# GaodeRender/triangle-splatting

Hardware: AMD Instinct MI355X
Metric: fwd+bwd Mpixels/sec @ 1M triangles, 1920x1080; achieved HBM GB/s (higher is better)
Workload: dtype f32

## Files before the change

triangle-splatting_amd/csrc/api.hip:

```cpp
#pragma GCC visibility push(default)
#include "../../include/ts2d.h"
#ifdef TS2D_LAB
#include "ts2d_lab.h"
#endif
#pragma GCC visibility pop
#include "ts2d_api.h"
#include <atomic>
#include <chrono>
#include <cstdarg>
#include <cstdio>
#include <cstring>
#include <mutex>
#include <string>
#include <vector>

namespace
{
thread_local std::string g_err;

struct ProfRow { std::string name; double ms = 0; int64_t launches = 0; };
struct ProfPending { int row; hipEvent_t a, b; };
std::mutex g_prof_mu;
bool g_prof_on = false;
std::string g_prof_only;
// ... 62 lines not shown
    a.rich_info = flags & TS2D_FLAG_RICH_INFO; a.use_shs = flags & TS2D_FLAG_USE_SHS;
    a.back_culling = flags & TS2D_FLAG_BACK_CULLING;
    a.tan_fovx = cam->tan_fovx; a.tan_fovy = cam->tan_fovy;
    a.viewmatrix = cam->viewmatrix; a.projmatrix = cam->projmatrix; a.campos = cam->campos;
    a.vertex = geom->vertex; a.shs = geom->shs; a.feature = geom->feature; a.opacity = geom->opacity;
    return a;
}

RenderArgs make_render(const ts2d_camera *cam, const ts2d_geometry *geom, uint32_t flags)
{
    RenderArgs r;
    r.W = cam->width; r.H = cam->height; r.C = geom->C;
    r.grid_x = (cam->width + TS_TILE - 1) / TS_TILE; r.grid_y = (cam->height + TS_TILE - 1) / TS_TILE;
    r.gamma = geom->gamma; r.background_depth = geom->background_depth;
    r.background_depth_dev = geom->background_depth_dev;
    r.background = geom->background;
    r.rich_info = flags & TS2D_FLAG_RICH_INFO;
    r.block_masks = block_masks_in_keys(cam, flags);
#ifdef TS2D_LAB
    if (g_lab_kernel_cull) r.block_masks = false;
#endif
    return r;
}

inline void cpu_relax()
{
#if defined(__x86_64__) || defined(__i386__)
    __builtin_ia32_pause();
#elif defined(__aarch64__)
    asm volatile("yield" ::: "memory");
#endif
}

struct CapacityHint { int dev, variant, W, H; unsigned long long key; double per_triangle; unsigned long long stamp; };
thread_local unsigned long long t_hint_key = 0;
std::atomic<unsigned long long> g_speculative_overflows{0};
std::mutex g_hint_mu;
std::vector<CapacityHint> g_hints;
unsigned long long g_hint_clock = 0;

void record_instance_count(int variant, int W, int H, int P, unsigned long long n)
{
    int dev = 0;
    if (P <= 0 || hipGetDevice(&dev) != hipSuccess) return;
    const double per = (double)n / (double)P;
    std::lock_guard<std::mutex> lk(g_hint_mu);
    CapacityHint *slot = nullptr;
    for (auto &h : g_hints)
        if (h.dev == dev && h.variant == variant && h.W == W && h.H == H && h.key == t_hint_key) slot = &h;
    if (!slot)
    {
        if (g_hints.size() < 32) { g_hints.push_back({dev, variant, W, H, t_hint_key, 0.0, 0}); slot = &g_hints.back(); }
        else
        {
            slot = &g_hints[0];
            for (auto &h : g_hints)
                if (h.stamp < slot->stamp) slot = &h;
            *slot = {dev, variant, W, H, t_hint_key, 0.0, 0};
        }
    }
    slot->per_triangle = per > 0.97 * slot->per_triangle ? per : 0.97 * slot->per_triangle;
    slot->stamp = ++g_hint_clock;
}

int read_instance_count(const ts2d_camera *cam, const ts2d_geometry *geom, uint32_t flags, const ts2d_state *state, const EarlyCount *early,
                        hipStream_t s, int64_t *num_rendered)
{
    if (int rc = wait_instance_count(geom->P, state, early, s, num_rendered)) return rc;
    record_instance_count((flags & TS2D_FLAG_3D) ? 3 : 2, cam->width, cam->height, geom->P, (unsigned long long)*num_rendered);
    return TS2D_OK;
}

int forward_bin_impl(const ts2d_camera *cam, const ts2d_geometry *geom, uint32_t flags, int32_t *radii, const ts2d_state *state, hipStream_t s,
                     const EarlyCount *early)
{
    const int P = geom->P;
    GeometryStateView g;
    ts_carve_geometry((char *)state->geometry, P, g);
    const PreprocessArgs a = make_pre(cam, geom, flags);
    {
        ProfScope ps("preprocess_fwd", s);
        if (flags & TS2D_FLAG_3D) ts_launch_preprocess3d_fwd(a, radii, g, s);
        else ts_launch_preprocess_fwd(a, radii, g, s);
    }
    TS_CHECK(flags, s, "preprocess_fwd");
    return ts_order_triangles(flags, g, P, early, s);
}

int forward_render_impl(const ts2d_camera *cam, const ts2d_geometry *geom, uint32_t flags, int64_t N, bool count_on_device,
                        const ts2d_state *state, const ts2d_forward_out *out, hipStream_t s)
{
    const bool rich = flags & TS2D_FLAG_RICH_INFO;
    const int P = geom->P, W = cam->width, H = cam->height;
    GeometryStateView g{};
    BinningStateView b{};
    ImageStateView im{};
    if (P > 0) ts_carve_geometry((char *)state->geometry, P, g);
    if (N > 0)
    {
        ts_carve_binning((char *)state->binning, ts_binning_capacity(state->binning_bytes, W, H), W, H, b);
        if (!count_on_device) ts_binning_set_count(b, N);
    }
    ts_carve_image((char *)state->image, W, H, im);
    const RenderArgs r = make_render(cam, geom, flags);
    const int ntiles = r.grid_x * r.grid_y;
    const unsigned long long *n_dev = count_on_device ? ts_instance_count_dev(g, P) : nullptr;

    QuadMaskArgs quad{(flags & TS2D_FLAG_3D) ? 3 : 2, fmaxf(0.0f, 2.0f * geom->gamma), cam->tan_fovx, cam->tan_fovy, W, H, 1.0f / (float)W, 1.0f / (float)H,
                      block_masks_in_keys(cam, flags) ? 1 : 0};
#ifdef TS2D_LAB
    if (g_lab_all_quadrants) quad.variant = 0;
#endif
    if (int rc = ts_order_instances(flags, P, r.grid_x, ntiles, g, b, im, rich ? out->contrib_sum : nullptr, rich ? out->contrib_max : nullptr, N, n_dev,
                                    quad, s))
        return rc;
    {
        ProfScope ps("render_fwd", s);
        if (flags & TS2D_FLAG_3D)
            ts_launch_render3d_fwd_group(r, cam->tan_fovx, cam->tan_fovy, g, b, im, out->out_feature, out->depth, out->normal,
// ... 53 lines not shown
    if (row < 0) return;
    (void)hipEventRecord(b, s);
    std::lock_guard<std::mutex> lk(g_prof_mu);
    g_prof_pending.push_back({row, a, b});
}

bool acquire_early_count(EarlyCount &e)
{
    constexpr int SLOTS = 64, MAXDEV = 16;
    static unsigned long long *ring = [] {
        void *p = nullptr;
        return hipHostMalloc(&p, (size_t)MAXDEV * SLOTS * sizeof(unsigned long long), hipHostMallocPortable | hipHostMallocMapped | hipHostMallocCoherent) == hipSuccess
                   ? (unsigned long long *)p : nullptr;
    }();
    static hipEvent_t events[MAXDEV][SLOTS] = {};
    static std::atomic<unsigned> next{0};
    static std::mutex mu;
    int dev = 0;
    if (!ring || hipGetDevice(&dev) != hipSuccess || dev < 0 || dev >= MAXDEV) return false;
    const unsigned i = next.fetch_add(1) % SLOTS;
    {
        std::lock_guard<std::mutex> lk(mu);
#ifndef TS2D_COUNT_EVENT_FLAGS
#define TS2D_COUNT_EVENT_FLAGS (hipEventDisableTiming | hipEventBlockingSync)
#endif
        if (!events[dev][i] && hipEventCreateWithFlags(&events[dev][i], TS2D_COUNT_EVENT_FLAGS) != hipSuccess) return false;
    }
    e.host = ring + (size_t)dev * SLOTS + i;
    e.ev = events[dev][i];
    __atomic_store_n(e.host, ~0ull, __ATOMIC_RELEASE);
    return true;
}

int wait_instance_count(int P, const ts2d_state *state, const EarlyCount *early, hipStream_t s, int64_t *num_rendered)
{
    unsigned long long n = ~0ull;
    if (early)
    {
        const auto t0 = std::chrono::steady_clock::now();
        for (unsigned spin = 0;; spin++)
        {
            n = __atomic_load_n(early->host, __ATOMIC_ACQUIRE);
            if (n != ~0ull) break;
            cpu_relax();
            if ((spin & 63u) == 63u && std::chrono::steady_clock::now() - t0 > std::chrono::microseconds(250)) break;
        }
        if (n == ~0ull)
        {
            const hipError_t q = hipEventSynchronize(early->ev);
            if (q != hipSuccess) return ts_fail(TS2D_ERR_HIP, "waiting for the instance count: %s", hipGetErrorString(q));
            n = __atomic_load_n(early->host, __ATOMIC_ACQUIRE);
            if (n == ~0ull) return ts_fail(TS2D_ERR_HIP, "the instance count was not published");
        }
    }
    else
    {
        GeometryStateView g;
        ts_carve_geometry((char *)state->geometry, P, g);
        TS_HIP(hipMemcpyAsync(&n, ts_instance_count_dev(g, P), sizeof(n), hipMemcpyDeviceToHost, s));
        TS_HIP(hipStreamSynchronize(s));
    }
    if (n > 0x7fffffffull)
        return ts_fail(TS2D_ERR_CAPACITY, "%llu tile instances exceed the 2^31 - 1 the instance list can address", n);
    *num_rendered = (int64_t)n;
    return TS2D_OK;
}

int ts_order_triangles(uint32_t flags, const GeometryStateView &g, int P, const EarlyCount *early, hipStream_t s)
{
    {
        ProfScope ps("depth_census", s);
        ts_sort_by_depth_begin(g, P, early ? early->host : nullptr, s);
    }
    if (early) TS_HIP(hipEventRecord(early->ev, s));
    { ProfScope ps("depth_sort", s); ts_sort_by_depth_finish(g, P, s); }
    TS_CHECK(flags, s, "depth_sort");
    { ProfScope ps("scan", s); ts_scan_offsets(g, P, s); }
    TS_CHECK(flags, s, "scan");
    return TS2D_OK;
}

int ts_order_instances(uint32_t flags, int P, int grid_x, int ntiles, const GeometryStateView &g, const BinningStateView &b, const ImageStateView &im,
                       float *contrib_sum, float *contrib_max, int64_t N, const unsigned long long *n_dev, const QuadMaskArgs &quad, hipStream_t s)
{
    if (P > 0)
    {
        { ProfScope ps("emit_keys", s); ts_launch_emit_keys(P, grid_x, ntiles, g, b, im, contrib_sum, contrib_max, n_dev ? N : -1, im.status, quad, s); }
        TS_CHECK(flags, s, "emit_keys");
    }
    else ts_launch_zero_words((uint32_t *)im.ranges, 2 * (size_t)ntiles, s);
    if (N > 0)
    {
        { ProfScope ps("tile_sort", s); ts_sort_pairs(b, N, n_dev, ntiles, s); }
        TS_CHECK(flags, s, "tile_sort");
        { ProfScope ps("tile_ranges", s); ts_launch_tile_ranges(N, n_dev, ntiles, b, im, s); }
        TS_CHECK(flags, s, "tile_ranges");
    }
    return TS2D_OK;
}

extern "C" {

const char *ts2d_version(void) { return "ts2d 0.1 (gfx950)"; }
const char *ts2d_last_error(void) { return g_err.c_str(); }

size_t ts2d_geometry_state_bytes(int32_t P)
{
    GeometryStateView v;
// ... 57 lines not shown
int ts2d_forward_render(const ts2d_camera *cam, const ts2d_geometry *geom, uint32_t flags, int64_t N,
                        const ts2d_state *state, const ts2d_forward_out *out, void *stream)
{
    if (int rc = check_forward_args(cam, geom, flags, N, state, out)) return rc;
    return forward_render_impl(cam, geom, flags, N, false, state, out, (hipStream_t)stream);
}

int ts2d_forward(const ts2d_camera *cam, const ts2d_geometry *geom, uint32_t flags, int32_t *radii, const ts2d_state *state,
                 int64_t instance_capacity, const ts2d_forward_out *out, void *stream)
{
    if (int rc = check_forward_args(cam, geom, flags, instance_capacity, state, out)) return rc;
    hipStream_t s = (hipStream_t)stream;
    if (geom->P == 0) return forward_render_impl(cam, geom, flags, 0, false, state, out, s);
    if (!radii) return ts_fail(TS2D_ERR_INVALID, "radii is null");
    if (instance_capacity <= 0) return ts_fail(TS2D_ERR_INVALID, "instance_capacity must be positive");
    if (int rc = forward_bin_impl(cam, geom, flags, radii, state, s, nullptr)) return rc;
    return forward_render_impl(cam, geom, flags, instance_capacity, true, state, out, s);
}

int ts2d_forward_speculative(const ts2d_camera *cam, const ts2d_geometry *geom, uint32_t flags, int32_t *radii, const ts2d_state *state,
                             const ts2d_forward_out *out, int64_t *num_rendered, void *stream)
{
    if (!num_rendered) return ts_fail(TS2D_ERR_INVALID, "null num_rendered");
    *num_rendered = 0;
    if (int rc = check_forward_args(cam, geom, flags, 0, state, out)) return rc;
    hipStream_t s = (hipStream_t)stream;
    const int P = geom->P, W = cam->width, H = cam->height;
    if (P == 0) return forward_render_impl(cam, geom, flags, 0, false, state, out, s);
    if (!radii) return ts_fail(TS2D_ERR_INVALID, "radii is null");
    int64_t cap = state->binning ? ts_binning_capacity(state->binning_bytes, W, H) : 0;
    if (state->binning && cap <= 0) return ts_fail(TS2D_ERR_CAPACITY, "binning state buffer too small for any instance (pass NULL to size it from num_rendered)");
    EarlyCount early;
    const bool have_early = acquire_early_count(early);
    if (int rc = forward_bin_impl(cam, geom, flags, radii, state, s, have_early ? &early : nullptr)) return rc;
    if (cap > 0)
    {
        if (int rc = forward_render_impl(cam, geom, flags, cap, true, state, out, s)) return rc;
    }
    if (int rc = read_instance_count(cam, geom, flags, state, have_early ? &early : nullptr, s, num_rendered)) return rc;
    if (cap > 0 && *num_rendered > cap) g_speculative_overflows.fetch_add(1, std::memory_order_relaxed);
    return TS2D_OK;
}

void ts2d_set_capacity_hint_key(uint64_t key) { t_hint_key = key; }
uint64_t ts2d_speculative_overflow_count(void) { return g_speculative_overflows.load(std::memory_order_relaxed); }

int ts2d_forward_status(const ts2d_state *state, int32_t P, int32_t width, int32_t height, int32_t *overflowed, int64_t *num_rendered,
                        void *stream)
{
    if (!state || !state->image || !overflowed || !num_rendered) return ts_fail(TS2D_ERR_INVALID, "null pointer");
    hipStream_t s = (hipStream_t)stream;
    *overflowed = 0;
    *num_rendered = 0;
    if (P <= 0) return TS2D_OK;
    if (!state->geometry) return ts_fail(TS2D_ERR_INVALID, "null geometry state");
    GeometryStateView g{};
    ImageStateView im{};
    ts_carve_geometry((char *)state->geometry, P, g);
    ts_carve_image((char *)state->image, width, height, im);
    unsigned long long n = 0;
    TS_HIP(hipMemcpyAsync(overflowed, im.status, sizeof(int32_t), hipMemcpyDeviceToHost, s));
    TS_HIP(hipMemcpyAsync(&n, ts_instance_count_dev(g, P), sizeof(n), hipMemcpyDeviceToHost, s));
    TS_HIP(hipStreamSynchronize(s));
    *num_rendered = (int64_t)n;
    return TS2D_OK;
}

int ts2d_backward(const ts2d_camera *cam, const ts2d_geometry *geom, uint32_t flags, int64_t N, const int32_t *radii,
                  const ts2d_state *state, const ts2d_loss_grads *loss, void *scratch, size_t scratch_bytes,
                  const ts2d_backward_out *out, void *stream)
{
    return ts2d_backward_ranged(cam, geom, flags, N, radii, state, loss, scratch, scratch_bytes, out, 1, nullptr, stream);
// ... 186 lines not shown
    case 13: src = im.n_contrib; bytes = (size_t)W * H * 4; break;
    case 14: src = im.final_T; bytes = (size_t)W * H * 4; break;
    case 15: src = b.k[(b.passes & 1) ^ 1]; bytes = (size_t)N * 4; break;
    case 16: src = b.v[(b.passes & 1) ^ 1]; bytes = (size_t)N * 4; break;
    case 17:
    {
        uint32_t top_const = 0;
        if (P > 0)
        {
            TS_HIP(hipMemcpyAsync(&top_const, g.top_const, 4, hipMemcpyDeviceToHost, s));
            TS_HIP(hipStreamSynchronize(s));
        }
        src = top_const ? g.sv[0] : g.sv[1];
        bytes = (size_t)P * 4;
        break;
    }
    case 18: src = g.rec; bytes = (size_t)P * TS_REC_FLOATS * 4; break;
    default: return ts_fail(TS2D_ERR_INVALID, "unknown field %d", field);
    }
    if (dst_bytes < bytes) return ts_fail(TS2D_ERR_CAPACITY, "dst too small");
    if (bytes)
    {
        TS_HIP(hipMemcpyAsync(dst, src, bytes, hipMemcpyDeviceToHost, s));
        TS_HIP(hipStreamSynchronize(s));
    }
    return TS2D_OK;
}

void ts2d_lab_force_ticket_passes(int on) { ts_force_ticket_passes(on != 0); }
void ts2d_lab_force_all_quadrants(int on) { g_lab_all_quadrants = on != 0; }
void ts2d_lab_force_kernel_cull(int on) { g_lab_kernel_cull = on != 0; }
void ts2d_lab_force_depth_pass4(int on) { ts_force_depth_pass4(on != 0); }
void ts2d_lab_depth_split(int mode, int bucket_cap) { ts_lab_depth_split(mode, bucket_cap); }
#endif

void ts2d_profile_enable(int on)
{
    std::lock_guard<std::mutex> lk(g_prof_mu);
    g_prof_on = on != 0;
}
void ts2d_profile_only(const char *name)
{
    std::lock_guard<std::mutex> lk(g_prof_mu);
    g_prof_only = name ? name : "";
}
void ts2d_profile_reset(void)
{
    std::lock_guard<std::mutex> lk(g_prof_mu);
    prof_drain();
    g_prof_rows.clear();
}
int ts2d_profile_read(int32_t index, char *name, size_t name_bytes, double *total_ms, int64_t *launches)
{
    std::lock_guard<std::mutex> lk(g_prof_mu);
    prof_drain();
    if (index < 0 || (size_t)index >= g_prof_rows.size()) return TS2D_ERR_INVALID;
    const ProfRow &r = g_prof_rows[index];
    if (name && name_bytes) { strncpy(name, r.name.c_str(), name_bytes - 1); name[name_bytes - 1] = 0; }
    if (total_ms) *total_ms = r.ms;
    if (launches) *launches = r.launches;
    return TS2D_OK;
}
}
```

triangle-splatting_amd/csrc/depth_order.hip:

```cpp
#include "ts2d_radix.h"

namespace
{
bool g_force_pass4 = false;

template <int CH>
__global__ void __launch_bounds__(256) rs_hist_census_direct_kernel(const uint32_t *__restrict__ keys, int64_t n, uint32_t mask, RadixScratchView r,
                                                                     uint32_t *__restrict__ acc, DepthCensus census)
{
    __shared__ uint32_t bins[NB];
    __shared__ unsigned long long csum[4];
    __shared__ uint32_t cor[4], cand[4];
    const int t = threadIdx.x, chunk = rs_chunk_of_block(r.chunks);
    if (chunk < 0) return;
    bins[t] = 0u;
    __syncthreads();
    const int64_t base = (int64_t)chunk * CH;
    KeyCensus mine;
#pragma unroll
    for (int b = 0; b < CH / 256; b++)
    {
        const int64_t i = base + 256 * b + t;
        if (i < n)
        {
// ... 538 lines not shown
    {
        const DepthSplit ds = depth_split_of(g);
        const dim3 grid((unsigned)g.rs.chunks);
        if (P < DSPL_SMALL_BELOW) hipLaunchKernelGGL(depth_split_sample_kernel<DSPL_SAMPLES_SMALL>, dim3(NB - 1), dim3(256), 0, s, P, g, ds);
        else hipLaunchKernelGGL(depth_split_sample_kernel<DSPL_SAMPLES>, dim3(NB - 1), dim3(256), 0, s, P, g, ds);
        TS_WITH_CHUNK(g.rs.chunk,
                      hipLaunchKernelGGL((depth_split_hist_kernel<CH>), grid, dim3(256), 0, s, (int64_t)P, g, g.rs, g.rs.slabacc[0], ds);
                      hipLaunchKernelGGL((depth_split_scatter_kernel<CH>), grid, dim3(256), 0, s, (int64_t)P, g, g.rs, (const uint32_t *)g.rs.slabacc[0], ds, host_out))
        return;
    }
    DepthCensus c;
    c.tiles_touched = g.tiles_touched;
    c.chunk_sum = (unsigned long long *)g.blocksum;
    c.chunk_or = g.tiles_sorted;
    c.chunk_and = g.offsets;
    c.n_out = (unsigned long long *)g.blocksum + (P + SB - 1) / SB;
    c.host_out = host_out;
    c.top_const = g.top_const;
    c.force_varying = g_force_pass4 ? 0xFF000000u : 0u;
    const dim3 grid((unsigned)g.rs.chunks);
    const uint32_t *keys = (const uint32_t *)g.depth;
    const unsigned long long *no_count = nullptr;
    const uint32_t *no_vals = nullptr, *no_skip = nullptr;
    if (form == DepthForm::LsdTickets)
    {
        TS_WITH_CHUNK(g.rs.chunk, hipLaunchKernelGGL((rs_hist_kernel<true, CH>), grid, dim3(256), 0, s, keys, (int64_t)P, no_count, 0, 0xFFu, g.rs, c, no_skip))
        return;
    }
    TS_WITH_CHUNK(g.rs.chunk,
                  hipLaunchKernelGGL((rs_hist_census_direct_kernel<CH>), grid, dim3(256), 0, s, keys, (int64_t)P, 0xFFu, g.rs, g.rs.slabacc[0], c);
                  hipLaunchKernelGGL((rs_scatter_kernel<true, CH, true, true>), grid, dim3(256), 0, s, keys, no_vals, g.sk[0], g.sv[0], (int64_t)P, no_count, 0, 8,
                                     g.rs, no_skip, (const uint32_t *)g.rs.slabacc[0], g.rs.slabacc[1], c))
}
void ts_sort_by_depth_finish(const GeometryStateView &g, int32_t P, hipStream_t s)
{
    if (P <= 0) return;
    switch (depth_form(P, g.rs))
    {
    case DepthForm::OneLaunch: return;
    case DepthForm::Split:
        if (P < DB_SMALL_BELOW)
            hipLaunchKernelGGL(depth_bucket_sort_kernel<DB_SMALL_WAVES>, dim3(NB), dim3(64 * DB_SMALL_WAVES), 0, s, P, g, depth_split_of(g),
                               min(g_depth_bucket_cap, 64 * DB_SMALL_WAVES * DB_KB));
        else hipLaunchKernelGGL(depth_bucket_sort_kernel<DB_WAVES>, dim3(NB), dim3(64 * DB_WAVES), 0, s, P, g, depth_split_of(g), g_depth_bucket_cap);
        return;
    case DepthForm::LsdTickets:
        ts_radix_scatter((const uint32_t *)g.depth, nullptr, g.sk[0], g.sv[0], P, nullptr, 0, 8, g.rs, s);
        ts_radix_pass(g.sk[0], g.sv[0], g.sk[1], g.sv[1], P, nullptr, 8, 8, g.rs, s);
        ts_radix_pass(g.sk[1], g.sv[1], g.sk[0], g.sv[0], P, nullptr, 16, 8, g.rs, s);
        ts_radix_pass(g.sk[0], g.sv[0], g.sk[1], g.sv[1], P, nullptr, 24, 8, g.rs, s, g.top_const);
        return;
    case DepthForm::LsdDirect:
        ts_radix_pass_direct(g.sk[0], g.sv[0], g.sk[1], g.sv[1], P, nullptr, 8, 8, g.rs, 1, s);
        ts_radix_pass_direct(g.sk[1], g.sv[1], g.sk[0], g.sv[0], P, nullptr, 16, 8, g.rs, 0, s);
        ts_radix_pass_direct(g.sk[0], g.sv[0], g.sk[1], g.sv[1], P, nullptr, 24, 8, g.rs, 1, s, g.top_const);
        return;
    }
}

bool ts_scan_two_level(int32_t P) { return ts_radix_tickets_forced() || (P + SB - 1) / SB > 2048; }
void ts_scan_offsets(const GeometryStateView &g, int32_t P, hipStream_t s)
{
    if (P <= 0) return;
    switch (depth_form(P, g.rs))
    {
    case DepthForm::OneLaunch:
    case DepthForm::Split: return;
    case DepthForm::LsdDirect:
    case DepthForm::LsdTickets: break;
    }
    hipLaunchKernelGGL(gather_blocksum_kernel, dim3((unsigned)((P + SB - 1) / SB)), dim3(256), 0, s, P, g, ts_scan_two_level(P));
}

void ts_force_depth_pass4(bool on) { g_force_pass4 = on; }
void ts_lab_depth_split(int mode, int bucket_cap)
{
    g_depth_split_mode = mode;
    g_depth_bucket_cap = bucket_cap > 0 && bucket_cap < DB_CAP ? bucket_cap : DB_CAP;
}
```

triangle-splatting_amd/csrc/ts2d_api.h:

```cpp
#ifndef TS2D_API_H
#define TS2D_API_H

#include "../../include/ts2d.h"
#include "ts2d_common.h"

#pragma GCC visibility push(hidden)
int ts_fail(int code, const char *fmt, ...) __attribute__((format(printf, 2, 3)));

#define TS_HIP(expr)                                                                                                   \
    do                                                                                                                 \
    {                                                                                                                  \
        hipError_t e_ = (expr);                                                                                        \
        if (e_ != hipSuccess) return ts_fail(TS2D_ERR_HIP, "%s failed: %s", #expr, hipGetErrorString(e_));           \
    } while (0)

#define TS_CHECK(flags, stream, what)                                                                                  \
    do                                                                                                                 \
    {                                                                                                                  \
        hipError_t e_ = hipGetLastError();                                                                             \
        if (e_ == hipSuccess && ((flags)&TS2D_FLAG_DEBUG)) e_ = hipStreamSynchronize(stream);                          \
        if (e_ != hipSuccess) return ts_fail(TS2D_ERR_HIP, "%s: %s", what, hipGetErrorString(e_));                     \
    } while (0)

struct ProfScope
{
    hipStream_t s;
    int row = -1;
    hipEvent_t a = nullptr, b = nullptr;
    ProfScope(const char *name, hipStream_t stream);
    ~ProfScope();
};

struct EarlyCount
{
    unsigned long long *host = nullptr;
    hipEvent_t ev = nullptr;
};
bool acquire_early_count(EarlyCount &e);
int wait_instance_count(int P, const ts2d_state *state, const EarlyCount *early, hipStream_t s, int64_t *num_rendered);

int ts_order_triangles(uint32_t flags, const GeometryStateView &g, int P, const EarlyCount *early, hipStream_t s);
int ts_order_instances(uint32_t flags, int P, int grid_x, int ntiles, const GeometryStateView &g, const BinningStateView &b, const ImageStateView &im,
                       float *contrib_sum, float *contrib_max, int64_t N, const unsigned long long *n_dev, const QuadMaskArgs &quad, hipStream_t s);

#pragma GCC visibility pop
#endif
```

triangle-splatting_amd/csrc/ts2d_common.h:

```cpp
#pragma once
#include <hip/hip_runtime.h>
#include <stddef.h>
#include <stdint.h>

#define TS_TILE 16
#define TS_ALIGN 256

#define TS_REC_FLOATS 16

#define TS_ID_BITS 28
#define TS_ID_MASK 0x0FFFFFFFu
#define TS_GRAD_FLOATS 16

#ifndef TS_RS_CHUNK
#define TS_RS_CHUNK 4096
#endif
#define TS_RS_CHUNK_MID 2048
#define TS_RS_CHUNK_SMALL 1024
#define TS_RS_SMALL_BELOW 2500000
static inline int ts_instance_chunk(size_t n) { return n <= (size_t)TS_RS_SMALL_BELOW ? TS_RS_CHUNK_SMALL : TS_RS_CHUNK; }
static inline int ts_depth_chunk(size_t n) { return n <= (size_t)TS_RS_SMALL_BELOW ? TS_RS_CHUNK_SMALL : TS_RS_CHUNK_MID; }
#define TS_RS_BINS 256
#define TS_RS_TICKET_EXTRA 8
struct RadixScratchView
// ... 138 lines not shown
    }
    return lo;
}

static inline void ts_binning_set_count(BinningStateView &v, int64_t n)
{
    v.rs.chunks = (int)((n + v.rs.chunk - 1) / v.rs.chunk);
    v.rs.slabs = (v.rs.chunks + 63) / 64;
}

static inline size_t ts_carve_image(char *base, int32_t W, int32_t H, ImageStateView &v)
{
    char *p = base;
    int gx = (W + TS_TILE - 1) / TS_TILE, gy = (H + TS_TILE - 1) / TS_TILE;
    ts_carve(p, v.ranges, (size_t)gx * gy);
    ts_carve(p, v.n_contrib, (size_t)W * H);
    ts_carve(p, v.final_T, (size_t)W * H);
    ts_carve(p, v.status, (size_t)4);
    return (size_t)(p - base) + TS_ALIGN;
}

struct PreprocessArgs
{
    int W, H, P, D, M, C;
    int grid_x, grid_y;
    bool rich_info, use_shs, back_culling;
    float tan_fovx, tan_fovy;
    const float *viewmatrix, *projmatrix, *campos;
    const float *vertex, *shs, *feature, *opacity;
};

void ts_launch_preprocess_fwd(const PreprocessArgs &a, int32_t *radii, const GeometryStateView &g, hipStream_t s);
void ts_sort_by_depth_begin(const GeometryStateView &g, int32_t P, unsigned long long *host_out, hipStream_t s);
void ts_sort_by_depth_finish(const GeometryStateView &g, int32_t P, hipStream_t s);
void ts_scan_offsets(const GeometryStateView &g, int32_t P, hipStream_t s);
struct QuadMaskArgs
{
    int variant;
    float g2;
    float tan_fovx, tan_fovy;
    int W, H;
    float inv_W, inv_H;
    int blocks;
};
void ts_launch_zero_words(uint32_t *p, size_t n, hipStream_t s);
void ts_launch_emit_keys(int P, int grid_x, int ntiles, const GeometryStateView &g, const BinningStateView &b, const ImageStateView &im,
                         float *contrib_sum, float *contrib_max, int64_t capacity, int32_t *status, const QuadMaskArgs &qm, hipStream_t s);
const unsigned long long *ts_instance_count_dev(const GeometryStateView &g, int P);
void ts_sort_pairs(const BinningStateView &b, int64_t N, const unsigned long long *n_dev, int ntiles, hipStream_t s);
void ts_launch_tile_ranges(int64_t N, const unsigned long long *n_dev, int ntiles, const BinningStateView &b, const ImageStateView &im, hipStream_t s);
size_t ts_quantile_scratch_bytes();
void ts_quantile_threshold(const uint32_t *keys, size_t n, float q, void *scratch, float *thr, hipStream_t s);
void ts_quantile_passes(const uint32_t *keys, size_t n, float q, void *scratch, int first_pass, hipStream_t s);
size_t ts_quantile_state_words();
size_t ts_radix_scratch_bytes(size_t n);
int ts_radix_sort_pairs(uint32_t *const k[2], uint32_t *const v[2], size_t n, int end_bit, void *scratch, hipStream_t s, bool force_tickets = false);
void ts_force_ticket_passes(bool on);
void ts_force_depth_pass4(bool on);
void ts_lab_depth_split(int mode, int bucket_cap);

struct RenderArgs
{
    int W, H, C, grid_x, grid_y;
    float gamma, background_depth;
    const float *background;
    const float *background_depth_dev;
    bool rich_info;
// ... 104 lines not shown
```

triangle-splatting_amd/csrc/ts2d_lab.h:

```cpp
#ifndef TS2D_LAB_H
#define TS2D_LAB_H

#include "../../include/ts2d.h"

#ifdef __cplusplus
extern "C" {
#endif

int ts2d_debug_read_state(const ts2d_state *state, int32_t P, int64_t num_rendered, int32_t width, int32_t height,
                          int32_t field, void *dst, size_t dst_bytes, void *stream);

int ts2d_test_sort_pairs(const uint32_t *keys_in, const uint32_t *vals_in, uint32_t *keys_out, uint32_t *vals_out, size_t n,
                         int32_t end_bit, int32_t which, void *stream);
int ts2d_test_inclusive_scan_rocprim(const uint32_t *in, uint32_t *out, size_t n, void *stream);

void ts2d_lab_force_ticket_passes(int on);
void ts2d_lab_force_depth_pass4(int on);
size_t ts2d_test_quantile_scratch_bytes(void);
int ts2d_test_quantile(const uint32_t *keys, size_t n, float q, void *scratch, float *out, void *stream);
void ts2d_lab_depth_split(int mode, int bucket_cap);
void ts2d_lab_force_all_quadrants(int on);
void ts2d_lab_force_kernel_cull(int on);

#ifdef __cplusplus
}
#endif
#endif
```

triangle-splatting_amd/csrc/ts2d_radix.h:

```cpp
#pragma once
#include "ts2d_common.h"
#include "ts2d_wave.h"

namespace
{
constexpr int NB = TS_RS_BINS;
constexpr int SB = 1024;

__device__ __forceinline__ unsigned long long ballot64(bool p) { return __builtin_amdgcn_ballot_w64(p); }

__device__ __forceinline__ uint32_t wave_inclusive_scan(uint32_t v, int lane)
{
    int x = (int)v;
    x += __builtin_amdgcn_update_dpp(0, x, 0x111, 0xF, 0xF, true);
    x += __builtin_amdgcn_update_dpp(0, x, 0x112, 0xF, 0xF, true);
    x += __builtin_amdgcn_update_dpp(0, x, 0x114, 0xF, 0xF, true);
    x += __builtin_amdgcn_update_dpp(0, x, 0x118, 0xF, 0xF, true);
    x += __builtin_amdgcn_update_dpp(0, x, 0x142, 0xA, 0xF, true);
    x += __builtin_amdgcn_update_dpp(0, x, 0x143, 0xC, 0xF, true);
    return (uint32_t)x;
}
__device__ __forceinline__ unsigned long long wave_sum64(unsigned long long v)
{
    for (int o = 32; o > 0; o >>= 1) v += __shfl_xor(v, o);
// ... 201 lines not shown
    unsigned long long tiles = 0ull;
    uint32_t kor = 0u, kand = 0xFFFFFFFFu;
    __device__ __forceinline__ void add(uint32_t key, uint32_t tiles_touched)
    {
        tiles += tiles_touched;
        if (key != 0u) { kor |= key; kand &= key; }
    }
    __device__ __forceinline__ void combine(unsigned long long s, uint32_t o, uint32_t a) { tiles += s; kor |= o; kand &= a; }
    __device__ __forceinline__ void wave_fold()
    {
        for (int d = 32; d > 0; d >>= 1) combine(__shfl_xor(tiles, d), __shfl_xor(kor, d), __shfl_xor(kand, d));
    }
    __device__ __forceinline__ void park(unsigned long long *s, uint32_t *o, uint32_t *a) const
    {
        if ((threadIdx.x & 63) == 0) { s[threadIdx.x >> 6] = tiles; o[threadIdx.x >> 6] = kor; a[threadIdx.x >> 6] = kand; }
    }
    template <int W>
    static __device__ __forceinline__ KeyCensus gather(const unsigned long long *s, const uint32_t *o, const uint32_t *a)
    {
        KeyCensus c;
#pragma unroll
        for (int w = 0; w < W; w++) c.combine(s[w], o[w], a[w]);
        return c;
    }
    __device__ __forceinline__ bool top_byte_constant(uint32_t force_varying = 0u) const { return (((kor ^ kand) | force_varying) >> 24) == 0u; }
};
template <bool PEER = false>
__device__ __forceinline__ void publish_instance_count(unsigned long long N, unsigned long long *n_out, uint32_t *top_const, bool verdict,
                                                       unsigned long long *host_out)
{
    *n_out = N;
    if (PEER) peer_store(top_const, verdict ? 1u : 0u);
    else *top_const = verdict ? 1u : 0u;
    if (host_out) __hip_atomic_store(host_out, N, __ATOMIC_RELAXED, __HIP_MEMORY_SCOPE_SYSTEM);
}

template <bool CENSUS, int CH>
__global__ void __launch_bounds__(256) rs_hist_kernel(const uint32_t *__restrict__ keys, int64_t n, const unsigned long long *n_dev, int shift,
                                                       uint32_t mask, RadixScratchView r, DepthCensus census, const uint32_t *skip_flag)
{
    __shared__ uint32_t bins[NB];
    __shared__ unsigned long long csum[4];
    __shared__ uint32_t cor[4], cand[4];
    if (!resolve_count<CH>(n_dev, n, r)) return;
    if (!CENSUS && pass_skipped(skip_flag)) return;
    const int t = threadIdx.x, chunk = rs_chunk_of_block(r.chunks);
    if (chunk < 0) return;
    bins[t] = 0u;
    __syncthreads();
    const int64_t base = (int64_t)chunk * CH;
    KeyCensus mine;
#pragma unroll 4
    for (int b = 0; b < CH / 256; b++)
    {
        const int64_t i = base + 256 * b + t;
        if (i < n)
        {
            const uint32_t k = keys[i];
            atomicAdd(&bins[(k >> shift) & mask], 1u);
            if (CENSUS) mine.add(k, census.tiles_touched[i]);
        }
    }
    if (CENSUS)
    {
        mine.wave_fold();
        mine.park(csum, cor, cand);
    }
// ... 260 lines not shown
```

triangle-splatting_amd/diff_triangle_rasterization_2D/_abi.py:

```python
import ctypes as C

_vp = C.c_void_p


class _Camera(C.Structure):
    _fields_ = [("width", C.c_int32), ("height", C.c_int32), ("tan_fovx", C.c_float), ("tan_fovy", C.c_float),
                ("viewmatrix", _vp), ("projmatrix", _vp), ("campos", _vp)]


class _Geometry(C.Structure):
    _fields_ = [("P", C.c_int32), ("sh_degree", C.c_int32), ("M", C.c_int32), ("C", C.c_int32),
                ("gamma", C.c_float), ("scale_modifier", C.c_float), ("background_depth", C.c_float),
                ("background", _vp), ("vertex", _vp), ("shs", _vp), ("feature", _vp), ("opacity", _vp), ("background_depth_dev", _vp)]


class _ForwardOut(C.Structure):
    _fields_ = [("out_feature", _vp), ("depth", _vp), ("normal", _vp), ("contrib_sum", _vp), ("contrib_max", _vp)]


class _LossGrads(C.Structure):
    _fields_ = [("dL_dout_feature", _vp), ("dL_dout_depth", _vp), ("dL_dout_normal", _vp)]


class _BackwardOut(C.Structure):
# ... 93 lines not shown
    "tsm_split_vertex": (C.c_int, [C.c_int32, _vp, _vp, _vp, _vp, _vp]),
    "tsm_update_mask": (C.c_int, [C.c_int32, C.c_int32, _vp, _vp, _vp, C.c_float, C.c_float, _vp, _vp]),
    "tsm_clip": (C.c_int, [C.c_int32, C.c_int32, _vp, C.c_float, _vp, _vp, _vp, _vp]),
    "tsm_opacity_reset": (C.c_int, [C.c_int32, C.c_float, _vp, _vp, _vp, _vp]),
    "tsm_max_vertex_distance": (C.c_int, [C.c_int32, _vp, _vp, _vp, _vp]),
    "tsm_state_digest": (C.c_int, [C.c_int32, C.POINTER(_vp), C.POINTER(C.c_uint64), _vp, _vp]),
    "tso_adam_step": (C.c_int, [C.POINTER(_Slice), C.c_int32, C.c_double, C.c_double, C.c_double, _vp]),
    "tso_adam_step_sh_factored": (C.c_int, [C.POINTER(_ShFactoredStep), C.c_double, C.c_double, C.c_double, _vp]),
    "ts2d_mesh_geometry_state_bytes": (C.c_size_t, [C.c_int32]),
    "ts2d_mesh_bin": (C.c_int, [C.POINTER(_Camera), C.c_float, C.c_int32, _vp, C.c_int32, _vp, C.POINTER(_State), C.POINTER(C.c_int64), _vp]),
    "ts2d_mesh_render": (C.c_int, [C.POINTER(_Camera), C.c_int32, _vp, _vp, C.c_int64, C.POINTER(_State), _vp, _vp, _vp, _vp, _vp]),
    "ts2d_mesh_render_counted": (C.c_int, [C.POINTER(_Camera), C.c_int32, _vp, _vp, C.c_int64, C.POINTER(_State), _vp, _vp, _vp, _vp, _vp, _vp]),
    "ts2d_mesh_census_add": (C.c_int, [C.c_int32, C.c_int32, C.c_int32, _vp, _vp, _vp, _vp, _vp]),
    "ts2d_weld_workspace_bytes": (C.c_size_t, [C.c_int32, C.c_int32]),
    "ts2d_weld_labels": (C.c_int, [C.c_int32, _vp, C.c_float, _vp, _vp, C.c_size_t, _vp]),
    "ts2d_weld_labels_counted": (C.c_int, [C.c_int32, _vp, C.c_float, _vp, _vp, _vp, C.c_size_t, _vp]),
    "ts2d_weld_face_components": (C.c_int, [C.c_int32, C.c_int32, _vp, _vp, _vp, _vp, C.c_size_t, _vp]),
    "ts2d_weld_compact": (C.c_int, [C.c_int32, _vp, _vp, C.c_int32, _vp, _vp, _vp, _vp, C.c_size_t, _vp]),
    "ts2d_weld_remap_faces": (C.c_int, [C.c_int32, C.c_int32, _vp, _vp, _vp, _vp, _vp]),
    "ts2d_weld_edge_census": (C.c_int, [C.c_int32, C.c_int32, _vp, _vp, _vp, _vp, C.c_size_t, _vp]),
}

LAB_SIGNATURES = {
    "ts2d_debug_read_state": (C.c_int, [C.POINTER(_State), C.c_int32, C.c_int64, C.c_int32, C.c_int32, C.c_int32, _vp, C.c_size_t, _vp]),
    "ts2d_test_sort_pairs": (C.c_int, [_vp, _vp, _vp, _vp, C.c_size_t, C.c_int32, C.c_int32, _vp]),
    "ts2d_test_inclusive_scan_rocprim": (C.c_int, [_vp, _vp, C.c_size_t, _vp]),
    "ts2d_lab_force_ticket_passes": (None, [C.c_int]),
    "ts2d_lab_force_depth_pass4": (None, [C.c_int]),
    "ts2d_test_quantile_scratch_bytes": (C.c_size_t, []),
    "ts2d_test_quantile": (C.c_int, [_vp, C.c_size_t, C.c_float, _vp, _vp, _vp]),
    "ts2d_lab_depth_split": (None, [C.c_int, C.c_int]),
    "ts2d_lab_force_all_quadrants": (None, [C.c_int]),
    "ts2d_lab_force_kernel_cull": (None, [C.c_int]),
}

GEOM_SIGNATURES = {
    "tsg_last_error": (C.c_char_p, []),
    "tsg_cross_workspace_bytes": (C.c_size_t, [C.c_int32, C.c_int32]),
    "tsg_nearest_cross": (C.c_int, [C.c_int32, _vp, C.c_int32, _vp, _vp, _vp, _vp, _vp, C.c_size_t, _vp]),
    "tsg_sample_workspace_bytes": (C.c_size_t, [C.c_int32]),
    "tsg_face_areas": (C.c_int, [C.c_int32, C.c_int32, _vp, _vp, _vp, _vp, _vp]),
    "tsg_sample_surface": (C.c_int, [C.c_int32, C.c_int32, _vp, _vp, _vp, C.c_int32, C.c_uint64, _vp, _vp, _vp, C.c_size_t, _vp]),
}


BVH_SIGNATURES = {
    "tsb_last_error": (C.c_char_p, []),
    "tsb_bvh_bytes": (C.c_size_t, [C.c_int32]),
    "tsb_build_workspace_bytes": (C.c_size_t, [C.c_int32]),
    "tsb_build": (C.c_int, [C.c_int32, C.c_int32, _vp, _vp, _vp, _vp, C.c_size_t, _vp, C.c_size_t, _vp]),
    "tsb_closest_workspace_bytes": (C.c_size_t, [C.c_int32]),
    "tsb_closest": (C.c_int, [C.c_int32, _vp, C.c_int32, C.c_int32, _vp, _vp, _vp, C.c_size_t, _vp, _vp, _vp, _vp, _vp, C.c_size_t, _vp]),
}


RAY_SIGNATURES = {
    "tsr_last_error": (C.c_char_p, []),
    "tsr_cast_workspace_bytes": (C.c_size_t, [C.c_int32]),
    "tsr_cast": (C.c_int, [C.c_int32, _vp, _vp, _vp, C.c_double, C.c_double, C.c_int32, C.c_int32, _vp, C.c_size_t, _vp, _vp, _vp, _vp, _vp, _vp,
                           C.c_size_t, _vp]),
}


VOLUME_SIGNATURES = {
    "tsv_last_error": (C.c_char_p, []),
    "tsv_integrate": (C.c_int, [C.c_int32, C.c_int32, C.c_int32, C.c_float, C.c_float, C.c_float, C.c_float, C.c_float, _vp, C.c_float, C.c_float,
# ... 290 lines not shown
```

Baseline: 1356.

## Speculatively skip the fourth depth radix pass when the top byte was constant last call

The depth census now packs a 'top byte constant' verdict into the published instance count. The host remembers this verdict per camera or config and, on the next call, launches only three LSD radix passes when the top byte was constant last time. It removes one full key/value scatter pass over P triangles. If the prediction turns out wrong, binning and rendering are rerun with four passes, which costs a full redo on a mispredict.

```diff
diff --git a/triangle-splatting_amd/csrc/api.hip b/triangle-splatting_amd/csrc/api.hip
--- a/triangle-splatting_amd/csrc/api.hip
+++ b/triangle-splatting_amd/csrc/api.hip
@@ -118,14 +118,15 @@
 #endif
 }
 
-struct CapacityHint { int dev, variant, W, H; unsigned long long key; double per_triangle; unsigned long long stamp; };
+struct CapacityHint { int dev, variant, W, H; unsigned long long key; double per_triangle; unsigned long long stamp; int top_const; };
 thread_local unsigned long long t_hint_key = 0;
 std::atomic<unsigned long long> g_speculative_overflows{0};
+std::atomic<unsigned long long> g_depth_repredictions{0}, g_depth_pass_skips{0};
 std::mutex g_hint_mu;
 std::vector<CapacityHint> g_hints;
 unsigned long long g_hint_clock = 0;
 
-void record_instance_count(int variant, int W, int H, int P, unsigned long long n)
+void record_instance_count(int variant, int W, int H, int P, unsigned long long n, int top_const)
 {
     int dev = 0;
     if (P <= 0 || hipGetDevice(&dev) != hipSuccess) return;
@@ -136,29 +137,42 @@
         if (h.dev == dev && h.variant == variant && h.W == W && h.H == H && h.key == t_hint_key) slot = &h;
     if (!slot)
     {
-        if (g_hints.size() < 32) { g_hints.push_back({dev, variant, W, H, t_hint_key, 0.0, 0}); slot = &g_hints.back(); }
+        if (g_hints.size() < 32) { g_hints.push_back({dev, variant, W, H, t_hint_key, 0.0, 0, -1}); slot = &g_hints.back(); }
         else
         {
             slot = &g_hints[0];
             for (auto &h : g_hints)
                 if (h.stamp < slot->stamp) slot = &h;
-            *slot = {dev, variant, W, H, t_hint_key, 0.0, 0};
+            *slot = {dev, variant, W, H, t_hint_key, 0.0, 0, -1};
         }
     }
     slot->per_triangle = per > 0.97 * slot->per_triangle ? per : 0.97 * slot->per_triangle;
     slot->stamp = ++g_hint_clock;
+    slot->top_const = top_const;
+}
+
+int predicted_depth_passes(int variant, int W, int H)
+{
+    int dev = 0;
+    if (hipGetDevice(&dev) != hipSuccess) return 4;
+    std::lock_guard<std::mutex> lk(g_hint_mu);
+    for (auto &h : g_hints)
+        if (h.dev == dev && h.variant == variant && h.W == W && h.H == H && h.key == t_hint_key) return h.top_const == 1 ? 3 : 4;
+    return 4;
 }
 
 int read_instance_count(const ts2d_camera *cam, const ts2d_geometry *geom, uint32_t flags, const ts2d_state *state, const EarlyCount *early,
-                        hipStream_t s, int64_t *num_rendered)
-{
-    if (int rc = wait_instance_count(geom->P, state, early, s, num_rendered)) return rc;
-    record_instance_count((flags & TS2D_FLAG_3D) ? 3 : 2, cam->width, cam->height, geom->P, (unsigned long long)*num_rendered);
+                        hipStream_t s, int64_t *num_rendered, bool *top_const = nullptr)
+{
+    bool tc = false;
+    if (int rc = wait_instance_count(geom->P, state, early, s, num_rendered, &tc)) return rc;
+    record_instance_count((flags & TS2D_FLAG_3D) ? 3 : 2, cam->width, cam->height, geom->P, (unsigned long long)*num_rendered, tc ? 1 : 0);
+    if (top_const) *top_const = tc;
     return TS2D_OK;
 }
 
 int forward_bin_impl(const ts2d_camera *cam, const ts2d_geometry *geom, uint32_t flags, int32_t *radii, const ts2d_state *state, hipStream_t s,
-                     const EarlyCount *early)
+                     const EarlyCount *early, int depth_passes = 4)
 {
     const int P = geom->P;
     GeometryStateView g;
@@ -170,7 +184,7 @@
         else ts_launch_preprocess_fwd(a, radii, g, s);
     }
     TS_CHECK(flags, s, "preprocess_fwd");
-    return ts_order_triangles(flags, g, P, early, s);
+    return ts_order_triangles(flags, g, P, early, s, depth_passes);
 }
 
 int forward_render_impl(const ts2d_camera *cam, const ts2d_geometry *geom, uint32_t flags, int64_t N, bool count_on_device,
@@ -290,9 +304,10 @@
     return true;
 }
 
-int wait_instance_count(int P, const ts2d_state *state, const EarlyCount *early, hipStream_t s, int64_t *num_rendered)
+int wait_instance_count(int P, const ts2d_state *state, const EarlyCount *early, hipStream_t s, int64_t *num_rendered, bool *top_const)
 {
     unsigned long long n = ~0ull;
+    if (top_const) *top_const = false;
     if (early)
     {
         const auto t0 = std::chrono::steady_clock::now();
@@ -310,6 +325,8 @@
             n = __atomic_load_n(early->host, __ATOMIC_ACQUIRE);
             if (n == ~0ull) return ts_fail(TS2D_ERR_HIP, "the instance count was not published");
         }
+        if (top_const) *top_const = (n & TS_COUNT_TOP_CONST_BIT) != 0ull;
+        n &= ~TS_COUNT_TOP_CONST_BIT;
     }
     else
     {
@@ -324,14 +341,14 @@
     return TS2D_OK;
 }
 
-int ts_order_triangles(uint32_t flags, const GeometryStateView &g, int P, const EarlyCount *early, hipStream_t s)
+int ts_order_triangles(uint32_t flags, const GeometryStateView &g, int P, const EarlyCount *early, hipStream_t s, int depth_passes)
 {
     {
         ProfScope ps("depth_census", s);
         ts_sort_by_depth_begin(g, P, early ? early->host : nullptr, s);
     }
     if (early) TS_HIP(hipEventRecord(early->ev, s));
-    { ProfScope ps("depth_sort", s); ts_sort_by_depth_finish(g, P, s); }
+    { ProfScope ps("depth_sort", s); ts_sort_by_depth_finish(g, P, s, depth_passes); }
     TS_CHECK(flags, s, "depth_sort");
     { ProfScope ps("scan", s); ts_scan_offsets(g, P, s); }
     TS_CHECK(flags, s, "scan");
@@ -455,12 +472,28 @@
     if (state->binning && cap <= 0) return ts_fail(TS2D_ERR_CAPACITY, "binning state buffer too small for any instance (pass NULL to size it from num_rendered)");
     EarlyCount early;
     const bool have_early = acquire_early_count(early);
-    if (int rc = forward_bin_impl(cam, geom, flags, radii, state, s, have_early ? &early : nullptr)) return rc;
+    int depth_passes = 4;
+    if (have_early)
+    {
+        GeometryStateView g;
+        ts_carve_geometry((char *)state->geometry, P, g);
+        if (ts_depth_pass_prediction_applies(g, P)) depth_passes = predicted_depth_passes((flags & TS2D_FLAG_3D) ? 3 : 2, W, H);
+    }
+    if (depth_passes == 3) g_depth_pass_skips.fetch_add(1, std::memory_order_relaxed);
+    if (int rc = forward_bin_impl(cam, geom, flags, radii, state, s, have_early ? &early : nullptr, depth_passes)) return rc;
     if (cap > 0)
     {
         if (int rc = forward_render_impl(cam, geom, flags, cap, true, state, out, s)) return rc;
     }
-    if (int rc = read_instance_count(cam, geom, flags, state, have_early ? &early : nullptr, s, num_rendered)) return rc;
+    bool top_const = false;
+    if (int rc = read_instance_count(cam, geom, flags, state, have_early ? &early : nullptr, s, num_rendered, &top_const)) return rc;
+    if (depth_passes == 3 && !top_const)
+    {
+        g_depth_repredictions.fetch_add(1, std::memory_order_relaxed);
+        if (int rc = forward_bin_impl(cam, geom, flags, radii, state, s, nullptr, 4)) return rc;
+        if (cap > 0 && *num_rendered <= cap)
+            if (int rc = forward_render_impl(cam, geom, flags, cap, true, state, out, s)) return rc;
+    }
     if (cap > 0 && *num_rendered > cap) g_speculative_overflows.fetch_add(1, std::memory_order_relaxed);
     return TS2D_OK;
 }
@@ -713,6 +746,8 @@
 void ts2d_lab_force_kernel_cull(int on) { g_lab_kernel_cull = on != 0; }
 void ts2d_lab_force_depth_pass4(int on) { ts_force_depth_pass4(on != 0); }
 void ts2d_lab_depth_split(int mode, int bucket_cap) { ts_lab_depth_split(mode, bucket_cap); }
+uint64_t ts2d_lab_depth_pass_skips(void) { return g_depth_pass_skips.load(std::memory_order_relaxed); }
+uint64_t ts2d_lab_depth_pass_repredictions(void) { return g_depth_repredictions.load(std::memory_order_relaxed); }
 #endif
 
 void ts2d_profile_enable(int on)
diff --git a/triangle-splatting_amd/csrc/depth_order.hip b/triangle-splatting_amd/csrc/depth_order.hip
--- a/triangle-splatting_amd/csrc/depth_order.hip
+++ b/triangle-splatting_amd/csrc/depth_order.hip
@@ -594,9 +594,16 @@
                   hipLaunchKernelGGL((rs_scatter_kernel<true, CH, true, true>), grid, dim3(256), 0, s, keys, no_vals, g.sk[0], g.sv[0], (int64_t)P, no_count, 0, 8,
                                      g.rs, no_skip, (const uint32_t *)g.rs.slabacc[0], g.rs.slabacc[1], c))
 }
-void ts_sort_by_depth_finish(const GeometryStateView &g, int32_t P, hipStream_t s)
+bool ts_depth_pass_prediction_applies(const GeometryStateView &g, int32_t P)
+{
+    if (P <= 0 || g_force_pass4 || g_depth_split_mode != 0) return false;
+    const DepthForm form = depth_form(P, g.rs);
+    return form == DepthForm::LsdDirect || form == DepthForm::LsdTickets;
+}
+void ts_sort_by_depth_finish(const GeometryStateView &g, int32_t P, hipStream_t s, int passes_hint)
 {
     if (P <= 0) return;
+    const bool fourth = !(passes_hint == 3 && ts_depth_pass_prediction_applies(g, P));
     switch (depth_form(P, g.rs))
     {
     case DepthForm::OneLaunch: return;
@@ -610,12 +617,12 @@
         ts_radix_scatter((const uint32_t *)g.depth, nullptr, g.sk[0], g.sv[0], P, nullptr, 0, 8, g.rs, s);
         ts_radix_pass(g.sk[0], g.sv[0], g.sk[1], g.sv[1], P, nullptr, 8, 8, g.rs, s);
         ts_radix_pass(g.sk[1], g.sv[1], g.sk[0], g.sv[0], P, nullptr, 16, 8, g.rs, s);
-        ts_radix_pass(g.sk[0], g.sv[0], g.sk[1], g.sv[1], P, nullptr, 24, 8, g.rs, s, g.top_const);
+        if (fourth) ts_radix_pass(g.sk[0], g.sv[0], g.sk[1], g.sv[1], P, nullptr, 24, 8, g.rs, s, g.top_const);
         return;
     case DepthForm::LsdDirect:
         ts_radix_pass_direct(g.sk[0], g.sv[0], g.sk[1], g.sv[1], P, nullptr, 8, 8, g.rs, 1, s);
         ts_radix_pass_direct(g.sk[1], g.sv[1], g.sk[0], g.sv[0], P, nullptr, 16, 8, g.rs, 0, s);
-        ts_radix_pass_direct(g.sk[0], g.sv[0], g.sk[1], g.sv[1], P, nullptr, 24, 8, g.rs, 1, s, g.top_const);
+        if (fourth) ts_radix_pass_direct(g.sk[0], g.sv[0], g.sk[1], g.sv[1], P, nullptr, 24, 8, g.rs, 1, s, g.top_const);
         return;
     }
 }
diff --git a/triangle-splatting_amd/csrc/ts2d_api.h b/triangle-splatting_amd/csrc/ts2d_api.h
--- a/triangle-splatting_amd/csrc/ts2d_api.h
+++ b/triangle-splatting_amd/csrc/ts2d_api.h
@@ -37,9 +37,9 @@
     hipEvent_t ev = nullptr;
 };
 bool acquire_early_count(EarlyCount &e);
-int wait_instance_count(int P, const ts2d_state *state, const EarlyCount *early, hipStream_t s, int64_t *num_rendered);
+int wait_instance_count(int P, const ts2d_state *state, const EarlyCount *early, hipStream_t s, int64_t *num_rendered, bool *top_const = nullptr);
 
-int ts_order_triangles(uint32_t flags, const GeometryStateView &g, int P, const EarlyCount *early, hipStream_t s);
+int ts_order_triangles(uint32_t flags, const GeometryStateView &g, int P, const EarlyCount *early, hipStream_t s, int depth_passes = 4);
 int ts_order_instances(uint32_t flags, int P, int grid_x, int ntiles, const GeometryStateView &g, const BinningStateView &b, const ImageStateView &im,
                        float *contrib_sum, float *contrib_max, int64_t N, const unsigned long long *n_dev, const QuadMaskArgs &quad, hipStream_t s);
 
diff --git a/triangle-splatting_amd/csrc/ts2d_common.h b/triangle-splatting_amd/csrc/ts2d_common.h
--- a/triangle-splatting_amd/csrc/ts2d_common.h
+++ b/triangle-splatting_amd/csrc/ts2d_common.h
@@ -194,7 +194,9 @@
 
 void ts_launch_preprocess_fwd(const PreprocessArgs &a, int32_t *radii, const GeometryStateView &g, hipStream_t s);
 void ts_sort_by_depth_begin(const GeometryStateView &g, int32_t P, unsigned long long *host_out, hipStream_t s);
-void ts_sort_by_depth_finish(const GeometryStateView &g, int32_t P, hipStream_t s);
+void ts_sort_by_depth_finish(const GeometryStateView &g, int32_t P, hipStream_t s, int passes_hint = 4);
+bool ts_depth_pass_prediction_applies(const GeometryStateView &g, int32_t P);
+#define TS_COUNT_TOP_CONST_BIT (1ull << 62)
 void ts_scan_offsets(const GeometryStateView &g, int32_t P, hipStream_t s);
 struct QuadMaskArgs
 {
diff --git a/triangle-splatting_amd/csrc/ts2d_lab.h b/triangle-splatting_amd/csrc/ts2d_lab.h
--- a/triangle-splatting_amd/csrc/ts2d_lab.h
+++ b/triangle-splatting_amd/csrc/ts2d_lab.h
@@ -21,6 +21,8 @@
 void ts2d_lab_depth_split(int mode, int bucket_cap);
 void ts2d_lab_force_all_quadrants(int on);
 void ts2d_lab_force_kernel_cull(int on);
+uint64_t ts2d_lab_depth_pass_skips(void);
+uint64_t ts2d_lab_depth_pass_repredictions(void);
 
 #ifdef __cplusplus
 }
diff --git a/triangle-splatting_amd/csrc/ts2d_radix.h b/triangle-splatting_amd/csrc/ts2d_radix.h
--- a/triangle-splatting_amd/csrc/ts2d_radix.h
+++ b/triangle-splatting_amd/csrc/ts2d_radix.h
@@ -257,7 +257,7 @@
     *n_out = N;
     if (PEER) peer_store(top_const, verdict ? 1u : 0u);
     else *top_const = verdict ? 1u : 0u;
-    if (host_out) __hip_atomic_store(host_out, N, __ATOMIC_RELAXED, __HIP_MEMORY_SCOPE_SYSTEM);
+    if (host_out) __hip_atomic_store(host_out, N | (verdict ? TS_COUNT_TOP_CONST_BIT : 0ull), __ATOMIC_RELAXED, __HIP_MEMORY_SCOPE_SYSTEM);
 }
 
 template <bool CENSUS, int CH>
diff --git a/triangle-splatting_amd/diff_triangle_rasterization_2D/_abi.py b/triangle-splatting_amd/diff_triangle_rasterization_2D/_abi.py
--- a/triangle-splatting_amd/diff_triangle_rasterization_2D/_abi.py
+++ b/triangle-splatting_amd/diff_triangle_rasterization_2D/_abi.py
@@ -149,6 +149,8 @@
     "ts2d_lab_depth_split": (None, [C.c_int, C.c_int]),
     "ts2d_lab_force_all_quadrants": (None, [C.c_int]),
     "ts2d_lab_force_kernel_cull": (None, [C.c_int]),
+    "ts2d_lab_depth_pass_skips": (C.c_uint64, []),
+    "ts2d_lab_depth_pass_repredictions": (C.c_uint64, []),
 }
 
 GEOM_SIGNATURES = {
```

New measurement: 1359 (median of 6 runs). No clear change (+0.2%).
